# petuum/poseidon

Measured on AMD Instinct MI355X. Metric: images/sec (whole node), higher is better.
Workload: dtype bf16; 1 GPU; model=alexnet, global_batch=256, input=3x227x227, parallelism=dp1, sfb=False, hipgraph=True

## Files before the change

### poseidon_amd/core/net.py

```python

from __future__ import annotations

from dataclasses import dataclass
from typing import Callable, Dict, List, Optional

import torch

from .blob import Blob
from .context import ctx
from .insert_splits import insert_splits
from .layer import Layer, create_layer
from ..ops import functional as ops
from ..proto import Message, spec
from ..proto.upgrade import net_needs_upgrade, upgrade_v0_net

TRAIN = spec.ENUMS["Phase"]["TRAIN"]
TEST = spec.ENUMS["Phase"]["TEST"]


def state_meets_rule(state: Message, rule: Message) -> bool:
    if rule.has("phase") and rule.phase != state.phase:
        return False
    if rule.has("min_level") and state.level < rule.min_level:
        return False
# ... 54 lines not shown
            param = upgrade_v0_net(param)
        filtered = filter_net(param, st)
        self.param = insert_splits(filtered)
        self.name = self.param.name or ""
        self._verbose = ctx().is_root() if verbose is None else verbose

        self.layers: List[Layer] = []
        self.layer_names: List[str] = []
        self.bottoms: List[List[Blob]] = []
        self.tops: List[List[Blob]] = []
        self.bottom_need_bwd: List[List[bool]] = []
        self.layer_need_bwd: List[bool] = []
        self.blobs: Dict[str, Blob] = {}
        self.params: List[ParamSpec] = []
        self._param_name_to_idx: Dict[str, int] = {}
        self.output_blob_names: List[str] = []
        self._loss_tops: List = []
        self._zero_mt = None
        self._repack_mt = None
        self._unpack_mt = None
        self._colsum_mt = None
        self._colsum_prev_key = None
        self._repack_key = None
        self._loss_marks: Dict[int, List] = {}
        self._lstream: List[int] = []
        self._producers: List[List[int]] = []
        self._consumers: List[List[int]] = []
        self._ms_nstreams = 0
        self._ms_pool = None
        self._fwd_ev = None
        self._bwd_ev = None

        self._build()
        self._build_stream_schedule()

    def _build(self) -> None:
        p = self.param
        available = set()
        blob_need: Dict[str, bool] = {}

        dims = list(p.input_dim)
        for i, name in enumerate(p.input):
            b = Blob(tuple(dims[4 * i:4 * i + 4]), name=name)
            self.blobs[name] = b
            available.add(name)
            blob_need[name] = False
# ... 291 lines not shown
            if prod_li is None:
                continue
            prod_lp = p.layers[prod_li]
            if prod_lp.enum_name("type") not in ("CONVOLUTION", "INNER_PRODUCT"):
                continue
            if len(prod_lp.top) != 1 or self.layers[prod_li].loss_weights[0] != 0.0:
                continue
            if any(prod_li < lj < li for lj in consumers.get(name, [])):
                continue
            self.layers[prod_li].fuse_relu = True
            relu.fused = True

    @property
    def learnable_params(self) -> List[ParamSpec]:
        return [ps for i, ps in enumerate(self.params) if ps.owner == i
                and ps.lr_mult != 0.0]

    def zero_param_diffs(self) -> None:
        owned = [ps.blob for i, ps in enumerate(self.params) if ps.owner == i]
        if owned and owned[0].data.is_cuda:
            extra = [t for l in self.layers
                     if hasattr(l, "extra_zero_buffers")
                     for t in l.extra_zero_buffers()]
            if self._zero_mt is None and all(
                    b.has_diff() and b.diff.dtype == torch.float32
                    and b.diff.is_contiguous() for b in owned):
                ts = [b.diff for b in owned] + extra
                self._zero_mt = (ops.zero_mt_prepare(ts), [id(t) for t in ts])
            if self._zero_mt is not None:
                mt, ids = self._zero_mt
                cur = [id(b.diff) for b in owned] + [id(t) for t in extra]
                if cur == ids:
                    ops.zero_mt_run(mt)
                    return
                self._zero_mt = None
            for t in extra:
                t.zero_()
        for b in owned:
            b.zero_diff()

    def _flush_deferred_unpacks(self) -> None:
        convs = [l for l in self.layers
                 if getattr(l, "_unpack_pending", False)]
        if not convs:
            return
        key = [(id(l._dwk_cache), id(l.blobs[0].diff), l._dwk_layout)
               for l in convs]
        if self._unpack_mt is None or self._unpack_mt[1] != key:
            self._unpack_mt = (ops.unpack_mt_prepare(
                [l._dwk_cache for l in convs],
                [l.blobs[0].diff for l in convs],
                [l.blobs[0].data.shape[1] for l in convs],
                [l.blobs[0].data.shape[2] for l in convs],
                [l.blobs[0].data.shape[3] for l in convs],
                [l._dwk_layout[0] for l in convs],
                [l._dwk_layout[1] for l in convs]), key)
        ops.unpack_mt_run(self._unpack_mt[0])
        for l in convs:
            l._unpack_pending = False
        pend = [(l, l._pending_colsum) for l in self.layers
                if getattr(l, "_pending_colsum", None) is not None]
        if pend:
            key = [(dy.data_ptr(), db.data_ptr(), tuple(dy.shape))
                   for _, (dy, db) in pend]
            key.append(ops.conv_policy_epoch())
            if self._colsum_mt is None or self._colsum_mt[1] != key:
                self._colsum_mt = (ops.colsum_mt_prepare(
                    [dy for _, (dy, db) in pend],
                    [db for _, (dy, db) in pend]), key)
            ops.colsum_mt_run(self._colsum_mt[0],
                              pend[0][1][0].dtype == torch.bfloat16)
            for l, _ in pend:
                l._pending_colsum = None

    def _maybe_mt_repack(self) -> None:
        if ctx().device != "cuda" or ctx().compute_dtype != torch.bfloat16:
            return
        convs = [l for l in self.layers
                 if l.type_name == "CONVOLUTION" and l.blobs
                 and l.blobs[0].data.is_cuda
                 and l.blobs[0].data.dtype == torch.float32]
        ips = [l for l in self.layers
               if l.type_name == "INNER_PRODUCT" and l.blobs
               and l.blobs[0].data.is_cuda
               and l.blobs[0].data.dtype == torch.float32]
        if not convs and not ips:
            return
        key = [id(l.blobs[0].data) for l in convs + ips]
        key.append(ops.conv_policy_epoch())
        if self._repack_mt is None or self._repack_key != key:
            masters, wks, wkTs, Gs, kw_lds, c_lds = [], [], [], [], [], []
            for l in convs:
                w = l.blobs[0].data
                Co, Cig, kh, kw = w.shape
                G = l.group
                x_shape = self.bottoms[self.layers.index(l)][0].shape
                plan = ops.conv_plan(x_shape, w.shape, l.stride, l.pad, G,
                                     bf16=True)
# ... 4 lines not shown
                                 device=w.device)
                wkT = torch.empty(G * kh * kw * Cig, Co // G,
                                  dtype=torch.bfloat16, device=w.device)
                l._wk_cache = (wk, wkT)
                masters.append(w)
                wks.append(wk)
                wkTs.append(wkT)
                Gs.append(G)
            for l in ips:
                w = l.blobs[0].data
                wk = torch.empty(l.N, l.K, dtype=torch.bfloat16,
                                 device=w.device)
                l._wk_cache = wk
                masters.append(w.view(l.N, l.K, 1, 1))
                wks.append(wk)
                wkTs.append(torch.empty(0, dtype=torch.bfloat16,
                                        device=w.device))
                Gs.append(1)
                kw_lds.append(1)
                c_lds.append(l.K)
            self._repack_mt = ops.repack_mt_prepare(masters, wks, wkTs, Gs,
                                                    kw_lds, c_lds)
            self._repack_key = key
        ops.repack_mt_run(self._repack_mt)

    def forward(self, start: int = 0, end: Optional[int] = None) -> float:
        end = len(self.layers) if end is None else end
        self._maybe_mt_repack()
        loss = 0.0
        for i in range(start, end):
            self.layers[i].forward(self.bottoms[i], self.tops[i])
            for (li, ti, w) in self._loss_tops:
                if li == i:
                    loss += w * float(self.tops[i][ti].data.sum().item())
        return loss

    def forward_async(self) -> torch.Tensor:
        dev = ctx().torch_device
        self._maybe_mt_repack()
        if self._ms_active():
            self._forward_ms()
            loss = torch.zeros((), dtype=torch.float32, device=dev)
            for (li, ti, w) in self._loss_tops:
                loss = loss + w * self.tops[li][ti].data.sum().to(torch.float32)
            return loss
        loss = torch.zeros((), dtype=torch.float32, device=dev)
# ... 121 lines not shown
```

### poseidon_amd/layers/common.py

```python

from __future__ import annotations

from typing import Optional, Tuple

import torch

from ..core.blob import Blob
from ..core.layer import Layer, register_layer
from ..core import filler
from ..ops import functional as ops


@register_layer("INNER_PRODUCT")
class InnerProductLayer(Layer):
    exact_num_bottom = 1
    exact_num_top = 1

    def layer_setup(self, bottom, top) -> None:
        ip = self.param.ensure("inner_product_param")
        self.N = int(ip.num_output)
        self.bias_term = bool(ip.bias_term)
        self.K = bottom[0].count // bottom[0].num
        dtype = torch.float64 if bottom[0].dtype == torch.float64 else torch.float32
        w = Blob((1, 1, self.N, self.K), dtype=dtype, name=f"{self.name}.weight")
        filler.fill(w, ip.weight_filler if ip.has("weight_filler") else None)
        self.blobs = [w]
        if self.bias_term:
            b = Blob((1, 1, 1, self.N), dtype=dtype, name=f"{self.name}.bias")
            filler.fill(b, ip.bias_filler if ip.has("bias_filler") else None)
            self.blobs.append(b)
        self.fuse_relu = False
        self._wk_cache = None
        self.sfb_active = False
        self.sfb_factors: Optional[Tuple[torch.Tensor, torch.Tensor]] = None

    def reshape(self, bottom, top) -> None:
        self.M = bottom[0].num
        assert bottom[0].count // self.M == self.K, \
            f"{self.name}: fan-in changed ({bottom[0].count // self.M} vs {self.K})"
        top[0].reshape(self.M, self.N)

    def forward(self, bottom, top) -> None:
        x = bottom[0].data.reshape(self.M, self.K)
        b = self.blobs[1].data.view(-1) if self.bias_term else None
        top[0].data = ops.linear_forward(
            x, self.blobs[0].data.view(self.N, self.K), b,
            fuse_relu=self.fuse_relu, w_shadow=self._wk_cache)

    def backward(self, top, propagate_down, bottom) -> None:
        x = bottom[0].data.reshape(self.M, self.K)
        dy = top[0].diff.reshape(self.M, self.N)
        need_dw = not self.sfb_active
        dw_acc = None
        import os as _os
        if (need_dw and dy.is_cuda
                and self.blobs[0].diff.dtype == torch.float32
                and _os.environ.get("PS_DW_ACC", "0") == "1"):
            dw_acc = self.blobs[0].diff.view(self.N, self.K)
        dx, dw, db = ops.linear_backward(
            x, self.blobs[0].data.view(self.N, self.K), dy,
            need_dx=propagate_down[0], need_dw=need_dw,
            has_bias=self.bias_term, w_shadow=self._wk_cache,
            dw_acc=dw_acc)
        if self.sfb_active:
            self.sfb_factors = (dy, x)
        elif dw_acc is None:
            self.blobs[0].diff.view(self.N, self.K).add_(dw)
        if self.bias_term:
            self.blobs[1].diff.view(-1).add_(db)
        if propagate_down[0]:
            bottom[0].diff = dx.reshape(bottom[0].shape)


@register_layer("CONCAT")
class ConcatLayer(Layer):
    min_bottom = 1
    exact_num_top = 1

    def layer_setup(self, bottom, top) -> None:
        cp = self.param.concat_param
        self.dim = int(cp.concat_dim) if cp is not None else 1

    def reshape(self, bottom, top) -> None:
        shape = list(bottom[0].shape)
        shape[self.dim] = sum(b.shape[self.dim] for b in bottom)
        top[0].reshape(shape)

    def forward(self, bottom, top) -> None:
        if self.dim == 1 and len(bottom[0].shape) == 4:
# ... 256 lines not shown
```

### poseidon_amd/layers/vision.py

```python

from __future__ import annotations

from typing import List

import torch
import torch.nn.functional as F

from ..core.blob import Blob
from ..core.layer import Layer, register_layer
from ..core import filler
from ..ops import functional as ops


def _pair(param, base: str, generic: str):
    h = getattr(param, f"{base}_h")
    w = getattr(param, f"{base}_w")
    if param.has(f"{base}_h") or param.has(f"{base}_w"):
        return int(h), int(w)
    g = getattr(param, generic)
    if g is None:
        raise ValueError(f"missing {generic} / {base}_h/w")
    return int(g), int(g)


# ... 15 lines not shown
        self._wk_cache = None
        self._dwk_cache = None
        self._dwk_packed = None
        self._dwk_layout = None
        self._unpack_pending = False
        self._dx_cache = {}
        self._pending_colsum = None
        self._last_dy_ptr = None
        self.bias_grad_by_consumer = False
        channels = bottom[0].channels
        assert channels % self.group == 0 and self.num_output % self.group == 0

        dtype = torch.float64 if bottom[0].dtype == torch.float64 else torch.float32
        w = Blob((self.num_output, channels // self.group,
                  self.kernel[0], self.kernel[1]), dtype=dtype,
                 name=f"{self.name}.weight")
        filler.fill(w, cp.weight_filler if cp.has("weight_filler") else None)
        self.blobs = [w]
        if self.bias_term:
            b = Blob((1, 1, 1, self.num_output), dtype=dtype,
                     name=f"{self.name}.bias")
            filler.fill(b, cp.bias_filler if cp.has("bias_filler") else None)
            self.blobs.append(b)

    def reshape(self, bottom: List[Blob], top: List[Blob]) -> None:
        n, c, h, w = bottom[0].shape
        ho = ops.conv_out_size(h, self.kernel[0], self.pad[0], self.stride[0])
        wo = ops.conv_out_size(w, self.kernel[1], self.pad[1], self.stride[1])
        for t in top:
            t.reshape(n, self.num_output, ho, wo)

    def forward(self, bottom: List[Blob], top: List[Blob]) -> None:
        w = self.blobs[0].data
        b = self.blobs[1].data.view(-1) if self.bias_term else None
        self._colT = []
        for bo, t in zip(bottom, top):
            y, colT = ops.conv2d_forward_ex(bo.data, w, b, self.stride,
                                            self.pad, self.group,
                                            fuse_relu=self.fuse_relu,
                                            cached=self._wk_cache)
            t.data = y
            self._colT.append(colT)

    def backward(self, top: List[Blob], propagate_down: List[bool],
                 bottom: List[Blob]) -> None:
        w = self.blobs[0].data
# ... 242 lines not shown
```

### poseidon_amd/ops/csrc/bindings.cpp

```cpp

#include <torch/extension.h>
#include <c10/hip/HIPStream.h>
#include <hip/hip_runtime.h>

#include <algorithm>
#include <atomic>
#include <cmath>
#include <cstdlib>
#include <utility>

#include "ps_api.h"
#include "ps_mt.h"

namespace {

using at::Tensor;

hipStream_t stream() { return c10::hip::getCurrentHIPStream().stream(); }

bool is_bf16(const Tensor& t) { return t.scalar_type() == at::kBFloat16; }

struct P {
  void* p;
  explicit P(const Tensor& t) : p(t.data_ptr()) {}
// ... 168 lines not shown
                      const c10::optional<Tensor>& bias, bool fuse_relu,
                      const c10::optional<Tensor>& w_shadow) {
  check_float_like(x, "x");
  auto xc = x.contiguous();
  auto wc = linear_weight(w, w_shadow, is_bf16(x));
  int M = xc.size(0), K = xc.size(1), N = wc.size(0);
  TORCH_CHECK(wc.size(1) == K, "linear: K mismatch");
  Tensor y = at::empty({M, N}, x.options());
  const float* bp = nullptr;
  Tensor bc;
  if (bias.has_value()) {
    bc = bias->contiguous();
    bp = bc.data_ptr<float>();
  }
  run_gemm(xc, wc, y, bp, M, N, K, K, K, N, 0, 0, 0, true, true, 1.0f, 0.0f,
           nullptr, nullptr, fuse_relu);
  return y;
}

std::vector<c10::optional<Tensor>> linear_backward(
    const Tensor& x, const Tensor& w, const Tensor& dy,
    bool need_dx, bool need_dw, bool has_bias,
    const c10::optional<Tensor>& w_shadow,
    const c10::optional<Tensor>& dw_acc) {
  check_float_like(dy, "dy");
  auto xc = x.contiguous();
  auto wc = linear_weight(w, w_shadow, is_bf16(dy));
  auto dyc = dy.contiguous();
  int M = xc.size(0), K = xc.size(1), N = wc.size(0);
  c10::optional<Tensor> dx, dw, db;
  if (need_dx) {
    Tensor t = at::empty({M, K}, x.options());
    run_gemm(dyc, wc, t, nullptr, M, K, N, N, K, K, 0, 0, 0, true, false,
             1.0f, 0.0f);
    dx = t;
  }
  if (need_dw) {
    Tensor t = dw_acc.has_value()
                   ? *dw_acc
                   : at::empty({N, K}, x.options().dtype(at::kFloat));
    TORCH_CHECK(t.scalar_type() == at::kFloat && t.is_contiguous());
    run_gemm(dyc, xc, t, nullptr, N, K, M, N, K, K, 0, 0, 0, false, false,
             1.0f, dw_acc.has_value() ? 1.0f : 0.0f);
    if (!dw_acc.has_value()) dw = t;
  }
  if (has_bias) {
    Tensor t = at::zeros({N}, x.options().dtype(at::kFloat));
    colsum_into(dyc, t.data_ptr<float>(), M, N);
    db = t;
  }
  return {dx, dw, db};
}

Tensor gemm_at_b(const Tensor& a, const Tensor& b) {
  check_float_like(a, "a");
  auto ac = a.contiguous();
  auto bc = b.contiguous();
  int M = ac.size(0), N = ac.size(1), K = bc.size(1);
  Tensor t = at::empty({N, K}, a.options().dtype(at::kFloat));
  run_gemm(ac, bc, t, nullptr, N, K, M, N, K, K, 0, 0, 0, false, false,
           1.0f, 0.0f);
  return t;
}


enum { PS_PACKED_OFF = 0, PS_PACKED_ON = 1, PS_PACKED_AUTO = -1 };

// ... 843 lines not shown
}

template <typename Chunk = ps::MTChunk, typename Desc, typename Extent>
std::vector<Tensor> mt_tables(const std::vector<Desc>& descs,
                              const Tensor& like, Extent extent) {
  std::vector<Chunk> chunks;
  for (size_t t = 0; t < descs.size(); ++t) {
    const std::pair<int64_t, int64_t> e = extent(descs[t]);
    for (int64_t off = 0; off < e.first; off += e.second)
      chunks.push_back({(int)t, off});
  }
  return {vec_to_dev(descs, like), vec_to_dev(chunks, like),
          at::scalar_tensor((int64_t)chunks.size())};
}

const auto mt_by_elts = [](const auto& d) {
  return std::pair<int64_t, int64_t>(d.n, ps::MT_CHUNK);
};

std::vector<Tensor> sgd_mt_prepare(std::vector<Tensor> ws,
                                   std::vector<Tensor> gs,
                                   std::vector<Tensor> hs,
                                   std::vector<double> lr_mults,
                                   std::vector<double> wds) {
  const size_t nt = ws.size();
  TORCH_CHECK(gs.size() == nt && hs.size() == nt && lr_mults.size() == nt &&
              wds.size() == nt, "sgd_mt_prepare: length mismatch");
  std::vector<ps::MTDesc> descs(nt);
  for (size_t t = 0; t < nt; ++t) {
    TORCH_CHECK(ws[t].is_cuda() && ws[t].is_contiguous() &&
                ws[t].scalar_type() == at::kFloat &&
                gs[t].is_contiguous() && hs[t].is_contiguous(),
                "sgd_mt_prepare: params must be contiguous f32 CUDA");
    int64_t n = ws[t].numel();
    TORCH_CHECK(gs[t].numel() == n && hs[t].numel() == n);
    descs[t] = {ws[t].data_ptr<float>(), gs[t].data_ptr<float>(),
                hs[t].data_ptr<float>(), n, (float)lr_mults[t],
                (float)wds[t]};
  }
  return mt_tables(descs, ws[0], mt_by_elts);
}

void sgd_mt_run(const Tensor& desc_dev, const Tensor& chunk_dev,
                int64_t nchunks, double lr, double mom,
                const c10::optional<Tensor>& lr_dev) {
  ps_sgd_mt(desc_dev.data_ptr(), chunk_dev.data_ptr(), (int)nchunks,
            (float)lr, (float)mom,
            lr_dev.has_value() ? lr_dev->data_ptr<float>() : nullptr,
            stream());
}

std::vector<Tensor> zero_mt_prepare(std::vector<Tensor> ts) {
  std::vector<ps::MTZeroDesc> descs(ts.size());
  for (size_t t = 0; t < ts.size(); ++t) {
    TORCH_CHECK(ts[t].is_cuda() && ts[t].is_contiguous() &&
                ts[t].scalar_type() == at::kFloat,
                "zero_mt_prepare: tensors must be contiguous f32 CUDA");
    descs[t] = {ts[t].data_ptr<float>(), ts[t].numel()};
  }
  return mt_tables(descs, ts[0], mt_by_elts);
}
// ... 35 lines not shown
  mt.push_back(at::empty({deterministic() ? nchunks * max_c : 0},
                         dys[0].options().dtype(at::kFloat)));
  return mt;
}

void colsum_mt_run(const Tensor& desc_dev, const Tensor& chunk_dev,
                   int64_t nchunks, bool bf16, int64_t max_c,
                   int64_t ntensors, const Tensor& scratch) {
  TORCH_CHECK(!deterministic() || scratch.numel() >= nchunks * max_c,
              "colsum_mt: table was prepared with deterministic mode off; "
              "prepare it again");
  ps_colsum_mt(desc_dev.data_ptr(), chunk_dev.data_ptr(), (int)nchunks,
               bf16 ? 1 : 0, (int)max_c, (int)ntensors,
               deterministic() ? scratch.data_ptr<float>() : nullptr,
               stream());
}

std::vector<Tensor> unpack_mt_prepare(std::vector<Tensor> dwks,
                                      std::vector<Tensor> dws,
                                      std::vector<int64_t> Cigs,
                                      std::vector<int64_t> khs,
                                      std::vector<int64_t> kws,
                                      std::vector<int64_t> kw_lds,
                                      std::vector<int64_t> c_lds) {
  const size_t nt = dwks.size();
  TORCH_CHECK((kw_lds.empty() && c_lds.empty()) ||
              (kw_lds.size() == nt && c_lds.size() == nt),
              "unpack_mt_prepare: layout length mismatch");
  std::vector<ps::MTUnpackDesc> descs(nt);
  for (size_t t = 0; t < nt; ++t) {
    TORCH_CHECK(dwks[t].is_cuda() && dwks[t].scalar_type() == at::kFloat &&
                dws[t].is_cuda() && dws[t].is_contiguous() &&
                dws[t].scalar_type() == at::kFloat,
                "unpack_mt_prepare: f32 CUDA tensors required");
    int Co = (int)dwks[t].size(0);
    int ldk = (int)dwks[t].size(1);
    int64_t n = dws[t].numel();
    TORCH_CHECK(n == (int64_t)Co * Cigs[t] * khs[t] * kws[t]);
    const int kw_ld = kw_lds.empty() ? (int)kws[t] : (int)kw_lds[t];
    const int c_ld = c_lds.empty() ? (int)Cigs[t] : (int)c_lds[t];
    TORCH_CHECK(kw_ld >= kws[t] && c_ld >= Cigs[t] &&
                (int64_t)khs[t] * kw_ld * c_ld <= ldk,
                "unpack_mt_prepare: khwc layout exceeds the dwk row");
    descs[t] = {dwks[t].data_ptr<float>(), dws[t].data_ptr<float>(), n,
                Co, (int)Cigs[t], (int)khs[t], (int)kws[t], ldk, kw_ld, c_ld};
  }
  return mt_tables(descs, dwks[0], mt_by_elts);
}

void unpack_mt_run(const Tensor& desc_dev, const Tensor& chunk_dev,
                   int64_t nchunks) {
  ps_unpack_mt(desc_dev.data_ptr(), chunk_dev.data_ptr(), (int)nchunks,
               stream());
}

std::vector<Tensor> repack_mt_prepare(std::vector<Tensor> masters,
                                      std::vector<Tensor> wks,
                                      std::vector<Tensor> wkTs,
                                      std::vector<int64_t> Gs,
                                      std::vector<int64_t> kw_lds,
                                      std::vector<int64_t> c_lds) {
  const size_t nt = masters.size();
  TORCH_CHECK((kw_lds.empty() && c_lds.empty()) ||
              (kw_lds.size() == nt && c_lds.size() == nt),
              "repack_mt_prepare: layout length mismatch");
  std::vector<ps::MTRepackDesc> descs(nt);
  for (size_t t = 0; t < nt; ++t) {
    const Tensor& m = masters[t];
// ... 161 lines not shown
```

### poseidon_amd/ops/csrc/ps_mt.h

```cpp
#pragma once
#include <cstdint>

#include "ps_conv_plan.h"

namespace ps {

constexpr int MT_CHUNK = 8192;

struct MTChunk {
  int t;
  int64_t off;
};

struct MTDesc {
  float* w;
  const float* g;
  float* h;
  int64_t n;
  float lr_mult;
  float wd;
};

struct MTZeroDesc {
  float* p;
  int64_t n;
};

struct MTRepackDesc {
  const float* src;
  void* wk;
  void* wkT;
  int64_t n;
  int Co, Cig, kh, kw, G, ldk;
  int kw_ld, c_ld;
};

struct MTUnpackDesc {
  const float* dwk;
  float* dw;
  int64_t n;
  int Co, Cig, kh, kw, ldk;
  int kw_ld, c_ld;
};

struct ColsumDesc {
  const void* dy;
  float* db;
  int64_t R;
  int64_t rows_per;
  int C;
};
struct ColsumChunk {
  int t;
  int64_t off;
};

}
```

### poseidon_amd/ops/csrc/sgd.hip

```cpp

#include "ps_common.h"
#include "ps_mt.h"

namespace ps {

__global__ void u64_inc_k(unsigned long long* p) { *p += 1; }

template <bool LRDEV>
__global__ void sgd_update_k(float* __restrict__ w, const float* __restrict__ g,
                             float* __restrict__ h, int64_t n, float lr_or_mult,
                             float mom, float wd, const float* __restrict__ lr_dev) {
  const float lr = LRDEV ? lr_dev[0] * lr_or_mult : lr_or_mult;
  int64_t i = ((int64_t)blockIdx.x * blockDim.x + threadIdx.x) * 4;
  int64_t stride = (int64_t)gridDim.x * blockDim.x * 4;
  for (; i + 4 <= n; i += stride) {
    f32x4 wv = *(f32x4*)&w[i];
    f32x4 gv = *(const f32x4*)&g[i];
    f32x4 hv = *(f32x4*)&h[i];
#pragma unroll
    for (int j = 0; j < 4; ++j) {
      hv[j] = mom * hv[j] + lr * (gv[j] + wd * wv[j]);
      wv[j] -= hv[j];
    }
    *(f32x4*)&w[i] = wv;
// ... 17 lines not shown
__global__ void nesterov_update_k(float* w, const float* g, float* h,
                                  int64_t n, float lr, float mom, float wd) {
  for (int64_t i = (int64_t)blockIdx.x * blockDim.x + threadIdx.x; i < n;
       i += (int64_t)gridDim.x * blockDim.x) {
    float h_old = h[i];
    float h_new = mom * h_old + lr * (g[i] + wd * w[i]);
    h[i] = h_new;
    w[i] -= (1.0f + mom) * h_new - mom * h_old;
  }
}

__global__ void adagrad_update_k(float* w, const float* g, float* h,
                                 int64_t n, float lr, float delta, float wd) {
  for (int64_t i = (int64_t)blockIdx.x * blockDim.x + threadIdx.x; i < n;
       i += (int64_t)gridDim.x * blockDim.x) {
    float gv = g[i] + wd * w[i];
    float hv = h[i] + gv * gv;
    h[i] = hv;
    w[i] -= lr * gv / (sqrtf(hv) + delta);
  }
}


template <bool LRDEV>
__global__ void sgd_mt_k(const MTDesc* __restrict__ descs,
                         const MTChunk* __restrict__ chunks, float lr_scalar,
                         float mom, const float* __restrict__ lr_dev) {
  const MTChunk ck = chunks[blockIdx.x];
  const MTDesc d = descs[ck.t];
  const float lr = (LRDEV ? lr_dev[0] : lr_scalar) * d.lr_mult;
  const float wd = d.wd;
  int64_t i = ck.off + (int64_t)threadIdx.x * 4;
#pragma unroll
  for (int it = 0; it < MT_CHUNK / (256 * 4); ++it, i += 256 * 4) {
    if (i + 4 <= d.n) {
      f32x4 wv = *(f32x4*)&d.w[i];
      f32x4 gv = *(const f32x4*)&d.g[i];
      f32x4 hv = *(f32x4*)&d.h[i];
#pragma unroll
      for (int j = 0; j < 4; ++j) {
        hv[j] = mom * hv[j] + lr * (gv[j] + wd * wv[j]);
        wv[j] -= hv[j];
      }
      *(f32x4*)&d.w[i] = wv;
      *(f32x4*)&d.h[i] = hv;
    } else if (i < d.n) {
      for (int64_t k = i; k < d.n; ++k) {
        float hv = mom * d.h[k] + lr * (d.g[k] + wd * d.w[k]);
        d.h[k] = hv;
        d.w[k] -= hv;
      }
    }
  }
}

__global__ void repack_mt_k(const MTRepackDesc* __restrict__ descs,
                            const MTChunk* __restrict__ chunks) {
  const MTChunk ck = chunks[blockIdx.x];
  const MTRepackDesc d = descs[ck.t];
  const int Cog = d.Co / d.G;
  const int Kg = d.kh * d.kw * d.Cig;
  const int KW = d.kw, KH = d.kh, Cig = d.Cig;
  if (KW == 1 && KH == 1 && d.G == 1 && !d.wkT && d.ldk == Cig) {
    typedef __bf16 bf16x4v __attribute__((ext_vector_type(4)));
    int64_t i = ck.off + (int64_t)threadIdx.x * 4;
#pragma unroll
    for (int it = 0; it < MT_CHUNK / (256 * 4); ++it, i += 256 * 4) {
      if (i + 4 <= d.n) {
        f32x4 v = *(const f32x4*)&d.src[i];
        bf16x4v o = {(__bf16)v[0], (__bf16)v[1], (__bf16)v[2], (__bf16)v[3]};
        *(bf16x4v*)((__bf16*)d.wk + i) = o;
      } else if (i < d.n) {
        for (int64_t k = i; k < d.n; ++k)
          ((__bf16*)d.wk)[k] = (__bf16)d.src[k];
      }
    }
    return;
  }
  for (int64_t i = ck.off + threadIdx.x;
       i < ck.off + MT_CHUNK && i < d.n; i += 256) {
    int kkw = (int)(i % KW);
    int64_t t = i / KW;
    int kkh = (int)(t % KH); t /= KH;
    int ci = (int)(t % Cig);
    int co = (int)(t / Cig);
    const float v = d.src[i];
    const int kg = (kkh * KW + kkw) * Cig + ci;
    ((__bf16*)d.wk)[(int64_t)co * d.ldk +
                    ps_khwc_col(kkh, kkw, ci, d.kw_ld, d.c_ld)] = (__bf16)v;
    if (d.wkT)
      ((__bf16*)d.wkT)[((int64_t)(co / Cog) * Kg + kg) * Cog + co % Cog] =
          (__bf16)v;
  }
}

__global__ void unpack_mt_k(const MTUnpackDesc* __restrict__ descs,
                            const MTChunk* __restrict__ chunks) {
  const MTChunk ck = chunks[blockIdx.x];
  const MTUnpackDesc d = descs[ck.t];
  const int KW = d.kw, KH = d.kh, Cig = d.Cig;
  for (int64_t i = ck.off + threadIdx.x;
       i < ck.off + MT_CHUNK && i < d.n; i += 256) {
    int kkw = (int)(i % KW);
    int64_t t = i / KW;
    int kkh = (int)(t % KH); t /= KH;
    int ci = (int)(t % Cig);
    int co = (int)(t / Cig);
    d.dw[i] += d.dwk[(int64_t)co * d.ldk +
                     ps_khwc_col(kkh, kkw, ci, d.kw_ld, d.c_ld)];
  }
}

__global__ void zero_mt_k(const MTZeroDesc* __restrict__ descs,
                          const MTChunk* __restrict__ chunks) {
  const MTChunk ck = chunks[blockIdx.x];
  const MTZeroDesc d = descs[ck.t];
  int64_t i = ck.off + (int64_t)threadIdx.x * 4;
  const f32x4 z = {0.f, 0.f, 0.f, 0.f};
#pragma unroll
  for (int it = 0; it < MT_CHUNK / (256 * 4); ++it, i += 256 * 4) {
    if (i + 4 <= d.n)
      *(f32x4*)&d.p[i] = z;
    else if (i < d.n)
      for (int64_t k = i; k < d.n; ++k) d.p[k] = 0.f;
  }
}

__global__ void f32_to_bf16_k(const float* src, __bf16* dst, int64_t n) {
  for (int64_t i = (int64_t)blockIdx.x * blockDim.x + threadIdx.x; i < n;
       i += (int64_t)gridDim.x * blockDim.x)
    dst[i] = (__bf16)src[i];
}
// ... 80 lines not shown
```

### poseidon_amd/ops/functional.py

```python

from __future__ import annotations

import math
import os
from typing import Optional, Tuple

import torch
import torch.nn.functional as F

_EXT = None
_EXT_ERR: Optional[str] = None


def _ext():
    global _EXT, _EXT_ERR
    if _EXT is None and _EXT_ERR is None:
        try:
            from . import _backend
            _EXT = _backend.load()
        except Exception as e:
            _EXT_ERR = str(e)
    if _EXT is None:
        raise RuntimeError(
            "poseidon_amd HIP extension is not built/loadable but a GPU op was "
# ... 24 lines not shown
    return _conv_policy_epoch


_deterministic_cpu = os.environ.get("PS_DETERMINISTIC", "0") not in ("", "0")


def set_deterministic(on: bool) -> None:
    global _deterministic_cpu, _conv_policy_epoch
    on = bool(on)
    if on == deterministic():
        return
    if ext_available():
        _ext().set_deterministic(on)
    _deterministic_cpu = on
    _conv_policy_epoch += 1
    from ..core.context import ctx
    ctx().deterministic = on


def deterministic() -> bool:
    if ext_available():
        return bool(_ext().deterministic())
    return _deterministic_cpu


def gemm_plan(M: int, N: int, K: int, a_klast: bool, b_klast: bool,
              bf16: bool) -> dict:
    return dict(_ext().gemm_plan(int(M), int(N), int(K), bool(a_klast),
                                 bool(b_klast), bool(bf16)))


def float_atomic_launches(reset: bool = False) -> int:
    if not ext_available():
        return 0
    return int(_ext().float_atomic_launches(bool(reset)))


def khwc_layout(Cg: int, kw: int, packed: bool) -> Tuple[int, int]:
    kw_ld, c_ld = _ext().khwc_layout(int(Cg), int(kw), bool(packed))
    return int(kw_ld), int(c_ld)


DGRAD_FWD_THRESHOLD_DEFAULT = 128 << 20


def set_dgrad_fwd_threshold(bytes_: int) -> None:
# ... 64 lines not shown
    if db is not None:
        db.add_(dy.sum(dim=(0, 2, 3)))
    return None



def linear_forward(x: torch.Tensor, w: torch.Tensor,
                   b: Optional[torch.Tensor],
                   fuse_relu: bool = False,
                   w_shadow: Optional[torch.Tensor] = None) -> torch.Tensor:
    if x.is_cuda:
        return _ext().linear_forward(x, w, b, fuse_relu, w_shadow)
    y = x.matmul(w.t())
    if b is not None:
        y = y + b
    if fuse_relu:
        y = F.relu(y)
    return y


def linear_backward(x: torch.Tensor, w: torch.Tensor, dy: torch.Tensor,
                    need_dx: bool, need_dw: bool, has_bias: bool,
                    w_shadow: Optional[torch.Tensor] = None,
                    dw_acc: Optional[torch.Tensor] = None):
    if dy.is_cuda:
        return _ext().linear_backward(x, w, dy, need_dx, need_dw, has_bias,
                                      w_shadow, dw_acc)
    dx = dy.matmul(w) if need_dx else None
    dw = dy.t().matmul(x) if need_dw else None
    db = dy.sum(dim=0) if has_bias else None
    return dx, dw, db


def gemm_at_b(a: torch.Tensor, b: torch.Tensor) -> torch.Tensor:
    if a.is_cuda:
        return _ext().gemm_at_b(a, b)
    return a.t().matmul(b)



def _unfold_pad(x, k, s, p, pad_value: float, Ho: int, Wo: int):
    H, W = x.shape[2], x.shape[3]
    far_h = max(p[0], (Ho - 1) * s[0] + k[0] - H - p[0])
    far_w = max(p[1], (Wo - 1) * s[1] + k[1] - W - p[1])
    xp = F.pad(x, (p[1], far_w, p[0], far_h), value=pad_value)
    return xp.unfold(2, k[0], s[0]).unfold(3, k[1], s[1])


def pool_max_forward(x, k, s, p):
    if x.is_cuda:
        return _ext().pool_max_forward(x, k[0], k[1], s[0], s[1], p[0], p[1])
    N, C, H, W = x.shape
# ... 311 lines not shown
    if dist_sq.is_cuda:
        return _ext().contrastive_forward(dist_sq, sim, float(margin),
                                          bool(legacy))
    m = torch.clamp(margin - (dist_sq if legacy else dist_sq.sqrt()), min=0)
    return torch.where(sim != 0, dist_sq, m if legacy else m * m)


def sgd_update(w: torch.Tensor, grad: torch.Tensor, hist: torch.Tensor,
               local_rate: float, momentum: float, decay: float,
               lr_dev=None) -> None:
    if w.is_cuda:
        if lr_dev is not None:
            _ext().sgd_update_lrdev(w, grad, hist, local_rate, momentum,
                                    decay, lr_dev)
        else:
            _ext().sgd_update(w, grad, hist, local_rate, momentum, decay)
        return
    gw = grad if decay == 0.0 else grad + decay * w
    hist.mul_(momentum).add_(gw, alpha=local_rate)
    w.sub_(hist)



def sgd_mt_prepare(ws, gs, hs, lr_mults, wds):
    d, c, n = _ext().sgd_mt_prepare(list(ws), list(gs), list(hs),
                                    [float(v) for v in lr_mults],
                                    [float(v) for v in wds])
    return d, c, int(n.item())


def sgd_mt_run(mt, lr: float, momentum: float, lr_dev=None) -> None:
    desc, chunk, nchunks = mt
    _ext().sgd_mt_run(desc, chunk, nchunks, float(lr), float(momentum),
                      lr_dev)


def conv_plan(x_shape, w_shape, stride, pad, groups: int, bf16: bool) -> dict:
    return _ext().conv_plan(list(x_shape), list(w_shape), list(stride),
                            list(pad), int(groups), bool(bf16))


def repack_mt_prepare(masters, wks, wkTs, Gs, kw_lds=(), c_lds=()):
    d, c, n = _ext().repack_mt_prepare(list(masters), list(wks), list(wkTs),
                                       [int(g) for g in Gs],
                                       [int(v) for v in kw_lds],
                                       [int(v) for v in c_lds])
    return d, c, int(n.item())


def repack_mt_run(mt) -> None:
    d, c, n = mt
    _ext().repack_mt_run(d, c, n)


def unpack_mt_prepare(dwks, dws, Cigs, khs, kws, kw_lds=(), c_lds=()):
    d, c, n = _ext().unpack_mt_prepare(list(dwks), list(dws), list(Cigs),
                                       list(khs), list(kws),
                                       [int(v) for v in kw_lds],
                                       [int(v) for v in c_lds])
    return d, c, int(n)


def unpack_mt_run(mt) -> None:
    d, c, n = mt
    _ext().unpack_mt_run(d, c, n)


def colsum_mt_prepare(dys, dbs):
    d, c, n, mc, nt, scratch = _ext().colsum_mt_prepare(list(dys), list(dbs))
    return d, c, int(n), int(mc), int(nt), scratch


def colsum_mt_run(mt, bf16: bool) -> None:
    d, c, n, mc, nt, scratch = mt
    _ext().colsum_mt_run(d, c, n, bf16, mc, nt, scratch)


def colsum_acc(dy, db) -> None:
    _ext().colsum_acc(dy, db)


def zero_mt_prepare(tensors):
# ... 97 lines not shown
```

### poseidon_amd/solver/solver.py

```python

from __future__ import annotations

import os
import time
from typing import Dict, List, Optional

import torch

from ..core.context import ctx
from ..core.net import Net, TRAIN, TEST
from ..core.blob import Blob
from ..ops import functional as ops
from ..parallel import comm
from ..proto import (Message, read_proto_text, read_proto_binary,
                     write_proto_binary)
from .sfb import SFBReducer, enable_sfb


def get_solver(param: Message, **kw) -> "SGDSolver":
    t = param.enum_name("solver_type")
    return {"SGD": SGDSolver, "NESTEROV": NesterovSolver,
            "ADAGRAD": AdaGradSolver}[t](param, **kw)


# ... 29 lines not shown
            if ps.owner == i and ps.lr_mult != 0.0:
                self.history[i] = torch.zeros_like(ps.blob.diff)

        self.distributed = comm.init_distributed()
        if self.distributed:
            comm.broadcast_params([ps for i, ps in enumerate(self.net.params)
                                   if ps.owner == i])
        self.reducer = comm.GradReducer(self.net) if self.distributed else None
        if not self.distributed and c.device == "cuda":
            for l in self.net.layers:
                if l.type_name == "CONVOLUTION":
                    l.defer_unpack = True
        want_sfb = c.use_sfb if use_sfb is None else use_sfb
        self.sfb = None
        if self.distributed and want_sfb:
            marked = enable_sfb(self.net, c.world_size)
            if marked:
                self.sfb = SFBReducer(
                    marked,
                    self.reducer.comm_stream if self.reducer.use_stream else None)
                if self.verbose:
                    print(f"[poseidon] SFB active on: "
                          f"{[l.name for l in marked]}", flush=True)

        self._net_outputs_rows: List[List[float]] = []
        self._net_outputs_cols: List[str] = []
        self._t0 = time.time()

        self._use_graph = False
        self._graph = None
        self._graph_loss = None
        self._lr_dev: Optional[torch.Tensor] = None
        self._staged_layers: list = []
        self._batch_staged = False
        self._mt = None

    def enable_graph(self) -> bool:
        c = ctx()
        if c.device != "cuda" or type(self) is not SGDSolver:
            return False
        if self.param.regularization_type == "L1":
            return False
        if self.distributed:
            import torch.distributed as dist
            if dist.get_backend() != "nccl":
                return False
        staged = []
        for layer in self.net.layers:
            t = layer.type_name
            if t in ("DATA", "IMAGE_DATA", "MEMORY_DATA", "WINDOW_DATA"):
                if not getattr(layer, "on_device", False):
                    return False
                staged.append(layer)
            if t == "DUMMY_DATA" and any(layer.refill):
                layer.forward(self.net.bottoms[self.net.layers.index(layer)],
                              self.net.tops[self.net.layers.index(layer)])
                layer.refill = [False] * len(layer.refill)
        for layer in staged:
            layer.external_staging = True
        self._staged_layers = staged
        self._batch_staged = False
        self._use_graph = True
        return True

    def _stage_inputs(self) -> None:
        for layer in self._staged_layers:
            layer.stage()

    def _release_staging(self) -> None:
        for layer in self._staged_layers:
            layer.external_staging = False
            layer.staged_ahead = self._batch_staged
        self._staged_layers = []
        self._batch_staged = False

    def _graph_body(self) -> torch.Tensor:
        loss = self.forward_backward()
        if not self._mt_update(0.0, lr_dev=self._lr_dev):
            for i, ps in enumerate(self.net.params):
                if ps.owner == i and ps.lr_mult != 0.0:
                    wd = float(self.param.weight_decay or 0.0) * ps.decay_mult
                    if self.distributed:
                        wd *= ctx().world_size
                    ops.sgd_update(ps.blob.data, ps.blob.diff,
                                   self.history[i], ps.lr_mult,
                                   float(self.param.momentum or 0.0),
                                   wd, lr_dev=self._lr_dev)
        return loss

    def _mt_update(self, rate: float, lr_dev=None) -> bool:
        if type(self) is not SGDSolver or ctx().device != "cuda":
            return False
        if self.param.regularization_type == "L1":
            return False
        items = [(i, ps) for i, ps in enumerate(self.net.params)
                 if ps.owner == i and ps.lr_mult != 0.0]
        if not items or not all(ps.blob.has_diff() for _, ps in items):
            return False
        key = [(id(ps.blob.data), id(ps.blob.diff), id(self.history[i]))
               for i, ps in items]
        if self._mt is None or self._mt[1] != key:
            wd0 = float(self.param.weight_decay or 0.0)
            if self.distributed:
                wd0 *= ctx().world_size
            mt = ops.sgd_mt_prepare(
                [ps.blob.data for _, ps in items],
                [ps.blob.diff for _, ps in items],
                [self.history[i] for i, _ in items],
                [ps.lr_mult for _, ps in items],
                [wd0 * ps.decay_mult for _, ps in items])
            self._mt = (mt, key)
        ops.sgd_mt_run(self._mt[0], rate,
                       float(self.param.momentum or 0.0), lr_dev)
        return True

    def _capture_graph(self) -> None:
        dev = ctx().torch_device
        self._lr_dev = torch.zeros(1, dtype=torch.float32, device=dev)
        self._lr_dev.fill_(self.get_learning_rate())
        saved = [(t, t.clone()) for i in self.history
                 for t in (self.net.params[i].blob.data, self.history[i])]
        counters = [(l, None if l._offset_dev is None
                     else l._offset_dev.clone())
                    for l in self.net.layers
                    if ops.deterministic() and hasattr(l, "_offset_dev")]
        if self._staged_layers and not self._batch_staged:
            self._stage_inputs()
            self._batch_staged = True
        side = torch.cuda.Stream()
        side.wait_stream(torch.cuda.current_stream())
        with torch.cuda.stream(side):
            for _ in range(3):
                self._graph_body()
        torch.cuda.current_stream().wait_stream(side)
        torch.cuda.synchronize()
        for t, t0 in saved:
            t.copy_(t0)
        del saved
        for l, t0 in counters:
            if l._offset_dev is not None:
                if t0 is None:
                    l._offset_dev.zero_()
                else:
                    l._offset_dev.copy_(t0)
        ok = True
        err: Optional[Exception] = None
        try:
            g = torch.cuda.CUDAGraph()
            with torch.cuda.graph(g):
                self._graph_loss = self._graph_body()
        except Exception as e:
            ok, err = False, e
            torch.cuda.synchronize()
        if self.distributed:
            import torch.distributed as dist
            flag = torch.tensor([1.0 if ok else 0.0], device=dev)
            dist.all_reduce(flag, op=dist.ReduceOp.MIN)
            ok = ok and float(flag.item()) > 0.0
        if not ok:
            raise RuntimeError(f"graph capture failed on some rank: {err}")
        self._graph = g

    def _step_graphed(self, iters: int) -> float:
        p = self.param
        last_loss = 0.0
        if self._graph is None:
            self._capture_graph()
        while iters > 0:
            if (p.snapshot and self.iter > 0
                    and self.iter % p.snapshot == 0):
                self.snapshot()
            if (p.test_interval and self.iter % p.test_interval == 0
                    and (self.iter > 0 or bool(p.test_initialization))):
                self.test_all()
            if self._staged_layers and not self._batch_staged:
                self._stage_inputs()
            self._batch_staged = False
            self._lr_dev.fill_(self.get_learning_rate())
            self._graph.replay()
            if p.display and self.iter % p.display == 0:
                last_loss = float(self._graph_loss.item())
                self._display(last_loss, self.get_learning_rate())
            self.iter += 1
            iters -= 1
        return last_loss

    @staticmethod
    def _load_net_param(param: Message) -> Message:
        if param.has("net_param"):
            return param.net_param
        if param.has("train_net_param"):
            return param.train_net_param
        path = param.net if param.has("net") else param.train_net
        if not path:
            raise ValueError("solver specifies no train net")
        return read_proto_text(path, "NetParameter")

    def _share_params(self, other: Net) -> None:
        by_name = {l.name: l for l in self.net.layers}
        for layer in other.layers:
            src = by_name.get(layer.name)
# ... 55 lines not shown
    def step(self, iters: int) -> float:
        if self._use_graph:
            try:
                return self._step_graphed(iters)
            except Exception as e:
                import sys
                print(f"[poseidon] graph capture failed ({e}); "
                      "falling back to eager", file=sys.stderr, flush=True)
                self._use_graph = False
                self._graph = None
                self._release_staging()
        last_loss = 0.0
        p = self.param
        while iters > 0:
            if (p.snapshot and self.iter > 0
                    and self.iter % p.snapshot == 0):
                self.snapshot()
            if (p.test_interval and self.iter % p.test_interval == 0
                    and (self.iter > 0 or bool(p.test_initialization))):
                self.test_all()
            loss_t = self.forward_backward()
            rate = self.get_learning_rate()
            if not self._mt_update(rate):
                for i, ps in enumerate(self.net.params):
                    if ps.owner == i and ps.lr_mult != 0.0:
                        self._apply_update(i, ps, rate)
            if p.display and self.iter % p.display == 0:
                last_loss = float(loss_t.item())
                self._display(last_loss, rate)
            self.iter += 1
            iters -= 1
        return last_loss

    def solve(self, resume_file: Optional[str] = None) -> None:
        p = self.param
        if resume_file:
            self.restore(resume_file)
        comm.barrier()
        self.step(int(p.max_iter) - self.iter)
        if bool(p.snapshot_after_train):
            self.snapshot()
        if p.test_interval:
            self.test_all()
        comm.barrier()

    def _display(self, loss: float, rate: float) -> None:
# ... 154 lines not shown
```

Before: 59200 images/sec.

## Fuse bf16 shadow refresh into SGD and overwrite weight grads instead of zeroing

The multi-tensor SGD kernel now also writes the bf16 shadow copy of each FC weight as it updates the fp32 master, so the next forward's repack can skip those FC layers. FC and deferred-unpack conv layers whose weight gradient is written whole each step now store dW directly (GEMM beta=0 into the diff, or an overwriting unpack) rather than zeroing the diff and accumulating into it. This cuts a zero pass, an add pass and a repack pass over the large AlexNet FC weights. In exchange it adds version and identity bookkeeping to decide when shadows are current, and it would break gradient accumulation if a layer's dW were written more than once per step.

```diff
diff --git a/poseidon_amd/core/net.py b/poseidon_amd/core/net.py
--- a/poseidon_amd/core/net.py
+++ b/poseidon_amd/core/net.py
@@ -100,6 +100,9 @@
         self._colsum_mt = None
         self._colsum_prev_key = None
         self._repack_key = None
+        self._repack_entries: List = []
+        self._repack_lite = None
+        self._fc_marks = None
         self._loss_marks: Dict[int, List] = {}
         self._lstream: List[int] = []
         self._producers: List[List[int]] = []
@@ -437,14 +440,20 @@
             extra = [t for l in self.layers
                      if hasattr(l, "extra_zero_buffers")
                      for t in l.extra_zero_buffers()]
+            skip = {id(l.blobs[0]) for l in self.layers
+                    if l.blobs and hasattr(l, "overwrites_dw")
+                    and l.overwrites_dw()}
+            zeroed = [b for b in owned if id(b) not in skip]
             if self._zero_mt is None and all(
                     b.has_diff() and b.diff.dtype == torch.float32
                     and b.diff.is_contiguous() for b in owned):
-                ts = [b.diff for b in owned] + extra
+                ts = [b.diff for b in zeroed] + extra
+                if not ts:
+                    return
                 self._zero_mt = (ops.zero_mt_prepare(ts), [id(t) for t in ts])
             if self._zero_mt is not None:
                 mt, ids = self._zero_mt
-                cur = [id(b.diff) for b in owned] + [id(t) for t in extra]
+                cur = [id(b.diff) for b in zeroed] + [id(t) for t in extra]
                 if cur == ids:
                     ops.zero_mt_run(mt)
                     return
@@ -459,8 +468,9 @@
                  if getattr(l, "_unpack_pending", False)]
         if not convs:
             return
-        key = [(id(l._dwk_cache), id(l.blobs[0].diff), l._dwk_layout)
-               for l in convs]
+        over = [l.overwrites_dw() for l in convs]
+        key = [(id(l._dwk_cache), id(l.blobs[0].diff), l._dwk_layout, o)
+               for l, o in zip(convs, over)]
         if self._unpack_mt is None or self._unpack_mt[1] != key:
             self._unpack_mt = (ops.unpack_mt_prepare(
                 [l._dwk_cache for l in convs],
@@ -469,7 +479,7 @@
                 [l.blobs[0].data.shape[2] for l in convs],
                 [l.blobs[0].data.shape[3] for l in convs],
                 [l._dwk_layout[0] for l in convs],
-                [l._dwk_layout[1] for l in convs]), key)
+                [l._dwk_layout[1] for l in convs], over), key)
         ops.unpack_mt_run(self._unpack_mt[0])
         for l in convs:
             l._unpack_pending = False
@@ -488,7 +498,32 @@
             for l, _ in pend:
                 l._pending_colsum = None
 
-    def _maybe_mt_repack(self) -> None:
+    def mark_fc_shadows_current(self, layers) -> None:
+        if self._repack_mt is None or not layers:
+            self._fc_marks = None
+            return
+        marks = [(l, l.blobs[0].data, l.blobs[0].data._version, l._wk_cache)
+                 for l in layers]
+        key = tuple(id(l) for l in layers)
+        if self._repack_lite is None or self._repack_lite[1] != key:
+            rest = [e for e in self._repack_entries
+                    if all(e[0] is not l for l in layers)]
+            mt = ops.repack_mt_prepare(*[[e[k] for e in rest]
+                                         for k in range(1, 7)]) \
+                if rest else None
+            self._repack_lite = (mt, key)
+        self._fc_marks = marks
+
+    def invalidate_fc_shadows(self) -> None:
+        self._fc_marks = None
+
+    def fc_shadows_current(self) -> bool:
+        marks = self._fc_marks
+        return (marks is not None and ops.fused_weight_tail()
+                and all(l.blobs[0].data is m and m._version == v
+                        and l._wk_cache is sh for l, m, v, sh in marks))
+
+    def _maybe_mt_repack(self, full: bool = False) -> None:
         if ctx().device != "cuda" or ctx().compute_dtype != torch.bfloat16:
             return
         convs = [l for l in self.layers
@@ -539,6 +574,15 @@
             self._repack_mt = ops.repack_mt_prepare(masters, wks, wkTs, Gs,
                                                     kw_lds, c_lds)
             self._repack_key = key
+            self._repack_entries = list(zip(convs + ips, masters, wks, wkTs,
+                                            Gs, kw_lds, c_lds))
+            self._repack_lite = None
+            self._fc_marks = None
+        if not full and self.fc_shadows_current():
+            if self._repack_lite[0] is not None:
+                ops.repack_mt_run(self._repack_lite[0])
+            return
+        self._fc_marks = None
         ops.repack_mt_run(self._repack_mt)
 
     def forward(self, start: int = 0, end: Optional[int] = None) -> float:
diff --git a/poseidon_amd/layers/common.py b/poseidon_amd/layers/common.py
--- a/poseidon_amd/layers/common.py
+++ b/poseidon_amd/layers/common.py
@@ -1,6 +1,7 @@
 
 from __future__ import annotations
 
+import os
 from typing import Optional, Tuple
 
 import torch
@@ -33,6 +34,14 @@
         self._wk_cache = None
         self.sfb_active = False
         self.sfb_factors: Optional[Tuple[torch.Tensor, torch.Tensor]] = None
+        self.dw_overwrite = False
+
+    def overwrites_dw(self) -> bool:
+        d = self.blobs[0]
+        return (self.dw_overwrite and not self.sfb_active
+                and ops.fused_weight_tail() and d.data.is_cuda
+                and d.data.dtype == torch.float32
+                and os.environ.get("PS_DW_ACC", "0") != "1")
 
     def reshape(self, bottom, top) -> None:
         self.M = bottom[0].num
@@ -57,14 +66,17 @@
                 and self.blobs[0].diff.dtype == torch.float32
                 and _os.environ.get("PS_DW_ACC", "0") == "1"):
             dw_acc = self.blobs[0].diff.view(self.N, self.K)
+        dw_out = None
+        if dw_acc is None and need_dw and self.overwrites_dw():
+            dw_out = self.blobs[0].diff.view(self.N, self.K)
         dx, dw, db = ops.linear_backward(
             x, self.blobs[0].data.view(self.N, self.K), dy,
             need_dx=propagate_down[0], need_dw=need_dw,
             has_bias=self.bias_term, w_shadow=self._wk_cache,
-            dw_acc=dw_acc)
+            dw_acc=dw_acc, dw_out=dw_out)
         if self.sfb_active:
             self.sfb_factors = (dy, x)
-        elif dw_acc is None:
+        elif dw_acc is None and dw_out is None:
             self.blobs[0].diff.view(self.N, self.K).add_(dw)
         if self.bias_term:
             self.blobs[1].diff.view(-1).add_(db)
diff --git a/poseidon_amd/layers/vision.py b/poseidon_amd/layers/vision.py
--- a/poseidon_amd/layers/vision.py
+++ b/poseidon_amd/layers/vision.py
@@ -61,6 +61,12 @@
                      name=f"{self.name}.bias")
             filler.fill(b, cp.bias_filler if cp.has("bias_filler") else None)
             self.blobs.append(b)
+
+    def overwrites_dw(self) -> bool:
+        return (getattr(self, "dw_overwrite", False)
+                and getattr(self, "defer_unpack", False)
+                and self._dwk_cache is not None
+                and ops.fused_weight_tail())
 
     def reshape(self, bottom: List[Blob], top: List[Blob]) -> None:
         n, c, h, w = bottom[0].shape
diff --git a/poseidon_amd/ops/csrc/bindings.cpp b/poseidon_amd/ops/csrc/bindings.cpp
--- a/poseidon_amd/ops/csrc/bindings.cpp
+++ b/poseidon_amd/ops/csrc/bindings.cpp
@@ -214,8 +214,11 @@
     const Tensor& x, const Tensor& w, const Tensor& dy,
     bool need_dx, bool need_dw, bool has_bias,
     const c10::optional<Tensor>& w_shadow,
-    const c10::optional<Tensor>& dw_acc) {
+    const c10::optional<Tensor>& dw_acc,
+    const c10::optional<Tensor>& dw_out) {
   check_float_like(dy, "dy");
+  TORCH_CHECK(!(dw_acc.has_value() && dw_out.has_value()),
+              "linear_backward: dw_acc and dw_out exclude each other");
   auto xc = x.contiguous();
   auto wc = linear_weight(w, w_shadow, is_bf16(dy));
   auto dyc = dy.contiguous();
@@ -228,13 +231,18 @@
     dx = t;
   }
   if (need_dw) {
-    Tensor t = dw_acc.has_value()
-                   ? *dw_acc
+    const bool own = !dw_acc.has_value() && !dw_out.has_value();
+    Tensor t = dw_acc.has_value() ? *dw_acc
+               : dw_out.has_value()
+                   ? *dw_out
                    : at::empty({N, K}, x.options().dtype(at::kFloat));
-    TORCH_CHECK(t.scalar_type() == at::kFloat && t.is_contiguous());
+    TORCH_CHECK(t.is_cuda() && t.scalar_type() == at::kFloat &&
+                t.is_contiguous() && t.dim() == 2 && t.size(0) == N &&
+                t.size(1) == K,
+                "linear_backward: dW target must be contiguous f32 [N,K]");
     run_gemm(dyc, xc, t, nullptr, N, K, M, N, K, K, 0, 0, 0, false, false,
              1.0f, dw_acc.has_value() ? 1.0f : 0.0f);
-    if (!dw_acc.has_value()) dw = t;
+    if (own) dw = t;
   }
   if (has_bias) {
     Tensor t = at::zeros({N}, x.options().dtype(at::kFloat));
@@ -1124,10 +1132,13 @@
                                    std::vector<Tensor> gs,
                                    std::vector<Tensor> hs,
                                    std::vector<double> lr_mults,
-                                   std::vector<double> wds) {
+                                   std::vector<double> wds,
+                                   std::vector<c10::optional<Tensor>> shadows) {
   const size_t nt = ws.size();
   TORCH_CHECK(gs.size() == nt && hs.size() == nt && lr_mults.size() == nt &&
               wds.size() == nt, "sgd_mt_prepare: length mismatch");
+  TORCH_CHECK(shadows.empty() || shadows.size() == nt,
+              "sgd_mt_prepare: shadows length mismatch");
   std::vector<ps::MTDesc> descs(nt);
   for (size_t t = 0; t < nt; ++t) {
     TORCH_CHECK(ws[t].is_cuda() && ws[t].is_contiguous() &&
@@ -1136,9 +1147,19 @@
                 "sgd_mt_prepare: params must be contiguous f32 CUDA");
     int64_t n = ws[t].numel();
     TORCH_CHECK(gs[t].numel() == n && hs[t].numel() == n);
+    void* shadow = nullptr;
+    if (!shadows.empty() && shadows[t].has_value()) {
+      const Tensor& sh = *shadows[t];
+      TORCH_CHECK(sh.is_cuda() && sh.is_contiguous() &&
+                  sh.scalar_type() == at::kBFloat16 && sh.numel() == n &&
+                  (uintptr_t)sh.data_ptr() % 8 == 0,
+                  "sgd_mt_prepare: a shadow must be contiguous bf16 CUDA "
+                  "with its tensor's element count");
+      shadow = sh.data_ptr();
+    }
     descs[t] = {ws[t].data_ptr<float>(), gs[t].data_ptr<float>(),
                 hs[t].data_ptr<float>(), n, (float)lr_mults[t],
-                (float)wds[t]};
+                (float)wds[t], shadow};
   }
   return mt_tables(descs, ws[0], mt_by_elts);
 }
@@ -1220,11 +1241,14 @@
                                       std::vector<int64_t> khs,
                                       std::vector<int64_t> kws,
                                       std::vector<int64_t> kw_lds,
-                                      std::vector<int64_t> c_lds) {
+                                      std::vector<int64_t> c_lds,
+                                      std::vector<bool> overwrites) {
   const size_t nt = dwks.size();
   TORCH_CHECK((kw_lds.empty() && c_lds.empty()) ||
               (kw_lds.size() == nt && c_lds.size() == nt),
               "unpack_mt_prepare: layout length mismatch");
+  TORCH_CHECK(overwrites.empty() || overwrites.size() == nt,
+              "unpack_mt_prepare: overwrites length mismatch");
   std::vector<ps::MTUnpackDesc> descs(nt);
   for (size_t t = 0; t < nt; ++t) {
     TORCH_CHECK(dwks[t].is_cuda() && dwks[t].scalar_type() == at::kFloat &&
@@ -1241,7 +1265,8 @@
                 (int64_t)khs[t] * kw_ld * c_ld <= ldk,
                 "unpack_mt_prepare: khwc layout exceeds the dwk row");
     descs[t] = {dwks[t].data_ptr<float>(), dws[t].data_ptr<float>(), n,
-                Co, (int)Cigs[t], (int)khs[t], (int)kws[t], ldk, kw_ld, c_ld};
+                Co, (int)Cigs[t], (int)khs[t], (int)kws[t], ldk, kw_ld, c_ld,
+                !overwrites.empty() && overwrites[t] ? 1 : 0};
   }
   return mt_tables(descs, dwks[0], mt_by_elts);
 }
diff --git a/poseidon_amd/ops/csrc/ps_mt.h b/poseidon_amd/ops/csrc/ps_mt.h
--- a/poseidon_amd/ops/csrc/ps_mt.h
+++ b/poseidon_amd/ops/csrc/ps_mt.h
@@ -19,6 +19,7 @@
   int64_t n;
   float lr_mult;
   float wd;
+  void* shadow;
 };
 
 struct MTZeroDesc {
@@ -41,6 +42,7 @@
   int64_t n;
   int Co, Cig, kh, kw, ldk;
   int kw_ld, c_ld;
+  int overwrite;
 };
 
 struct ColsumDesc {
diff --git a/poseidon_amd/ops/csrc/sgd.hip b/poseidon_amd/ops/csrc/sgd.hip
--- a/poseidon_amd/ops/csrc/sgd.hip
+++ b/poseidon_amd/ops/csrc/sgd.hip
@@ -63,6 +63,8 @@
 }
 
 
+typedef __bf16 bf16x4v __attribute__((ext_vector_type(4)));
+
 template <bool LRDEV>
 __global__ void sgd_mt_k(const MTDesc* __restrict__ descs,
                          const MTChunk* __restrict__ chunks, float lr_scalar,
@@ -71,6 +73,7 @@
   const MTDesc d = descs[ck.t];
   const float lr = (LRDEV ? lr_dev[0] : lr_scalar) * d.lr_mult;
   const float wd = d.wd;
+  __bf16* const sh = (__bf16*)d.shadow;
   int64_t i = ck.off + (int64_t)threadIdx.x * 4;
 #pragma unroll
   for (int it = 0; it < MT_CHUNK / (256 * 4); ++it, i += 256 * 4) {
@@ -85,11 +88,18 @@
       }
       *(f32x4*)&d.w[i] = wv;
       *(f32x4*)&d.h[i] = hv;
+      if (sh) {
+        bf16x4v o = {(__bf16)wv[0], (__bf16)wv[1], (__bf16)wv[2],
+                     (__bf16)wv[3]};
+        *(bf16x4v*)(sh + i) = o;
+      }
     } else if (i < d.n) {
       for (int64_t k = i; k < d.n; ++k) {
         float hv = mom * d.h[k] + lr * (d.g[k] + wd * d.w[k]);
         d.h[k] = hv;
-        d.w[k] -= hv;
+        const float wn = d.w[k] - hv;
+        d.w[k] = wn;
+        if (sh) sh[k] = (__bf16)wn;
       }
     }
   }
@@ -103,7 +113,6 @@
   const int Kg = d.kh * d.kw * d.Cig;
   const int KW = d.kw, KH = d.kh, Cig = d.Cig;
   if (KW == 1 && KH == 1 && d.G == 1 && !d.wkT && d.ldk == Cig) {
-    typedef __bf16 bf16x4v __attribute__((ext_vector_type(4)));
     int64_t i = ck.off + (int64_t)threadIdx.x * 4;
 #pragma unroll
     for (int it = 0; it < MT_CHUNK / (256 * 4); ++it, i += 256 * 4) {
@@ -147,8 +156,9 @@
     int kkh = (int)(t % KH); t /= KH;
     int ci = (int)(t % Cig);
     int co = (int)(t / Cig);
-    d.dw[i] += d.dwk[(int64_t)co * d.ldk +
-                     ps_khwc_col(kkh, kkw, ci, d.kw_ld, d.c_ld)];
+    const float v = d.dwk[(int64_t)co * d.ldk +
+                          ps_khwc_col(kkh, kkw, ci, d.kw_ld, d.c_ld)];
+    d.dw[i] = d.overwrite ? v : d.dw[i] + v;
   }
 }
 
diff --git a/poseidon_amd/ops/functional.py b/poseidon_amd/ops/functional.py
--- a/poseidon_amd/ops/functional.py
+++ b/poseidon_amd/ops/functional.py
@@ -70,6 +70,18 @@
     if ext_available():
         return bool(_ext().deterministic())
     return _deterministic_cpu
+
+
+_fused_weight_tail = os.environ.get("PS_WEIGHT_TAIL", "1") not in ("", "0")
+
+
+def set_fused_weight_tail(on: bool) -> None:
+    global _fused_weight_tail
+    _fused_weight_tail = bool(on)
+
+
+def fused_weight_tail() -> bool:
+    return _fused_weight_tail
 
 
 def gemm_plan(M: int, N: int, K: int, a_klast: bool, b_klast: bool,
@@ -180,12 +192,19 @@
 def linear_backward(x: torch.Tensor, w: torch.Tensor, dy: torch.Tensor,
                     need_dx: bool, need_dw: bool, has_bias: bool,
                     w_shadow: Optional[torch.Tensor] = None,
-                    dw_acc: Optional[torch.Tensor] = None):
+                    dw_acc: Optional[torch.Tensor] = None,
+                    dw_out: Optional[torch.Tensor] = None):
     if dy.is_cuda:
         return _ext().linear_backward(x, w, dy, need_dx, need_dw, has_bias,
-                                      w_shadow, dw_acc)
+                                      w_shadow, dw_acc, dw_out)
     dx = dy.matmul(w) if need_dx else None
     dw = dy.t().matmul(x) if need_dw else None
+    if dw is not None and dw_out is not None:
+        dw_out.copy_(dw)
+        dw = None
+    elif dw is not None and dw_acc is not None:
+        dw_acc.add_(dw)
+        dw = None
     db = dy.sum(dim=0) if has_bias else None
     return dx, dw, db
 
@@ -543,10 +562,12 @@
 
 
 
-def sgd_mt_prepare(ws, gs, hs, lr_mults, wds):
+def sgd_mt_prepare(ws, gs, hs, lr_mults, wds, shadows=None):
     d, c, n = _ext().sgd_mt_prepare(list(ws), list(gs), list(hs),
                                     [float(v) for v in lr_mults],
-                                    [float(v) for v in wds])
+                                    [float(v) for v in wds],
+                                    list(shadows) if shadows is not None
+                                    else [])
     return d, c, int(n.item())
 
 
@@ -574,11 +595,13 @@
     _ext().repack_mt_run(d, c, n)
 
 
-def unpack_mt_prepare(dwks, dws, Cigs, khs, kws, kw_lds=(), c_lds=()):
+def unpack_mt_prepare(dwks, dws, Cigs, khs, kws, kw_lds=(), c_lds=(),
+                      overwrites=()):
     d, c, n = _ext().unpack_mt_prepare(list(dwks), list(dws), list(Cigs),
                                        list(khs), list(kws),
                                        [int(v) for v in kw_lds],
-                                       [int(v) for v in c_lds])
+                                       [int(v) for v in c_lds],
+                                       [bool(v) for v in overwrites])
     return d, c, int(n)
 
 
diff --git a/poseidon_amd/solver/solver.py b/poseidon_amd/solver/solver.py
--- a/poseidon_amd/solver/solver.py
+++ b/poseidon_amd/solver/solver.py
@@ -75,6 +75,7 @@
                 if self.verbose:
                     print(f"[poseidon] SFB active on: "
                           f"{[l.name for l in marked]}", flush=True)
+        self._mark_dw_overwrite()
 
         self._net_outputs_rows: List[List[float]] = []
         self._net_outputs_cols: List[str] = []
@@ -87,6 +88,30 @@
         self._staged_layers: list = []
         self._batch_staged = False
         self._mt = None
+        self._shadow_layers: list = []
+
+    def _mark_dw_overwrite(self) -> None:
+        net = self.net
+        if ctx().device != "cuda":
+            return
+        users: Dict[int, int] = {}
+        for ps in net.params:
+            users[ps.owner] = users.get(ps.owner, 0) + 1
+        for idx, ps in enumerate(net.params):
+            layer = net.layers[ps.layer_idx]
+            if ps.param_idx != 0 or layer.type_name not in (
+                    "INNER_PRODUCT", "CONVOLUTION"):
+                continue
+            w = ps.blob.data
+            ok = (ps.owner == idx and users[idx] == 1 and ps.lr_mult != 0.0
+                  and net.layer_need_bwd[ps.layer_idx]
+                  and w.is_cuda and w.dtype == torch.float32
+                  and w.is_contiguous()
+                  and not getattr(layer, "sfb_active", False))
+            if layer.type_name == "CONVOLUTION":
+                ok = (ok and getattr(layer, "defer_unpack", False)
+                      and len(net.bottoms[ps.layer_idx]) == 1)
+            layer.dw_overwrite = ok
 
     def enable_graph(self) -> bool:
         c = ctx()
@@ -130,6 +155,7 @@
     def _graph_body(self) -> torch.Tensor:
         loss = self.forward_backward()
         if not self._mt_update(0.0, lr_dev=self._lr_dev):
+            self.net.invalidate_fc_shadows()
             for i, ps in enumerate(self.net.params):
                 if ps.owner == i and ps.lr_mult != 0.0:
                     wd = float(self.param.weight_decay or 0.0) * ps.decay_mult
@@ -150,8 +176,22 @@
                  if ps.owner == i and ps.lr_mult != 0.0]
         if not items or not all(ps.blob.has_diff() for _, ps in items):
             return False
-        key = [(id(ps.blob.data), id(ps.blob.diff), id(self.history[i]))
-               for i, ps in items]
+        shadows, covered = [], []
+        for _, ps in items:
+            layer = self.net.layers[ps.layer_idx]
+            sh = getattr(layer, "_wk_cache", None)
+            if (ops.fused_weight_tail() and ps.param_idx == 0
+                    and layer.type_name == "INNER_PRODUCT"
+                    and isinstance(sh, torch.Tensor)
+                    and sh.dtype == torch.bfloat16
+                    and sh.numel() == ps.blob.data.numel()):
+                shadows.append(sh)
+                covered.append(layer)
+            else:
+                shadows.append(None)
+        key = [(id(ps.blob.data), id(ps.blob.diff), id(self.history[i]),
+                id(sh) if sh is not None else 0)
+               for (i, ps), sh in zip(items, shadows)]
         if self._mt is None or self._mt[1] != key:
             wd0 = float(self.param.weight_decay or 0.0)
             if self.distributed:
@@ -161,11 +201,19 @@
                 [ps.blob.diff for _, ps in items],
                 [self.history[i] for i, _ in items],
                 [ps.lr_mult for _, ps in items],
-                [wd0 * ps.decay_mult for _, ps in items])
+                [wd0 * ps.decay_mult for _, ps in items],
+                shadows if covered else None)
             self._mt = (mt, key)
         ops.sgd_mt_run(self._mt[0], rate,
                        float(self.param.momentum or 0.0), lr_dev)
+        self._shadow_layers = covered
+        self.net.mark_fc_shadows_current(covered)
         return True
+
+    def _refresh_fc_shadows(self) -> None:
+        if self._shadow_layers:
+            self.net._maybe_mt_repack(full=True)
+            self.net.mark_fc_shadows_current(self._shadow_layers)
 
     def _capture_graph(self) -> None:
         dev = ctx().torch_device
@@ -190,6 +238,7 @@
         for t, t0 in saved:
             t.copy_(t0)
         del saved
+        self._refresh_fc_shadows()
         for l, t0 in counters:
             if l._offset_dev is not None:
                 if t0 is None:
@@ -230,6 +279,8 @@
                 self._stage_inputs()
             self._batch_staged = False
             self._lr_dev.fill_(self.get_learning_rate())
+            if self._shadow_layers and not self.net.fc_shadows_current():
+                self._refresh_fc_shadows()
             self._graph.replay()
             if p.display and self.iter % p.display == 0:
                 last_loss = float(self._graph_loss.item())
@@ -331,6 +382,7 @@
             loss_t = self.forward_backward()
             rate = self.get_learning_rate()
             if not self._mt_update(rate):
+                self.net.invalidate_fc_shadows()
                 for i, ps in enumerate(self.net.params):
                     if ps.owner == i and ps.lr_mult != 0.0:
                         self._apply_update(i, ps, rate)
```

After: 61400 images/sec, median of 6. 1.04x the previous value.
